# pymoc/pymoc

Measured on AMD Instinct MI355X. Metric: column-timesteps/sec (ensemble) at nz=100, higher is better.
Workload: dtype f64; 1 GPU; BASELINE configs[1]: 1024 independent Columns x nz=100 fp64 per GPU, static wA, do_conv on odd members, dt=30 d (pymoc_amd.configs.config2); columns_per_gpu=1024, nz=100, kernel=k_column_steps<64,2,6,true,true>, parallelism=ensemble sharded over 1 GPU(s), RCCL gather (root) of the final state

## Files before the change

### pymoc_amd/csrc/column.hip.h

```cpp
#pragma once
#include <type_traits>
#include "common.hip.h"

namespace pm {

template <int P>
struct ColGrid {
  double z[P];
  double dz[P];
  double dzc[P];
  double rdz[P], rdzc[P];
  double rdz_l[P], rdzc_l[P];
};
template <int P>
struct ColRegs {
  double b[P];
  double kap[P];
  double area[P];
  double dAk[P];
  double rarea[P];
  double rarea_l[P];
  double area_u, rarea_u, rarea_lu;
};

template <int P>
__device__ __forceinline__ void load_levels(double (&out)[P], const double *__restrict__ row,
                                            int lg, int nz, int lvl0 = 0) {
  if constexpr (P == 2) {
    if (lvl0 == 0 && (nz & 1) == 0 && (((unsigned long long)row) & 15ull) == 0ull) {
      const int i0 = lg * 2 < nz - 2 ? lg * 2 : nz - 2;
      const double2 v = *reinterpret_cast<const double2 *>(row + i0);
      out[0] = v.x;
      out[1] = v.y;
      return;
    }
  }
#pragma unroll
  for (int p = 0; p < P; ++p) {
    const int i = lvl0 + lg * P + p;
    out[p] = row[i < nz ? i : nz - 1];
  }
}

template <int P>
__device__ __forceinline__ double level_value(const double (&x)[P], int j) {
  const int jl = __builtin_amdgcn_readfirstlane(j / P);
  const int jp = __builtin_amdgcn_readfirstlane(j % P);
  double out = 0.;
#pragma unroll
  for (int p = 0; p < P; ++p) {
    const int lo = __builtin_amdgcn_readlane(__double2loint(x[p]), jl);
    const int hi = __builtin_amdgcn_readlane(__double2hiint(x[p]), jl);
    const double v = __hiloint2double(hi, lo);
    out = (p == 0 || jp == p) ? v : out;
  }
  return out;
}

__device__ __forceinline__ double lane_value(double x, int lane) {
  const int lo = __builtin_amdgcn_readlane(__double2loint(x), lane);
  const int hi = __builtin_amdgcn_readlane(__double2hiint(x), lane);
  return __hiloint2double(hi, lo);
}

template <int P>
struct ConvCache {
  unsigned long long mask[P];
  double zconv;
  bool valid = false;
};

template <int G, int P>
__device__ __forceinline__ bool col_convect(double (&b)[P], const double (&z)[P],
                                            double bs, double N2min, int lg, int lane,
                                            int nz, const double *__restrict__ zg,
                                            ConvCache<P> *cache = nullptr) {
  const unsigned long long gm = group_mask<G>(lane);
  bool ind[P];
  unsigned long long im[P];
  unsigned long long anym = 0ull;
#pragma unroll
  for (int p = 0; p < P; ++p) {
    const int i = lg * P + p;
    ind[p] = (i < nz) && (b[p] > bs);
    im[p] = __builtin_amdgcn_ballot_w64(ind[p]);
    anym |= im[p] & gm;
  }
  if (__builtin_expect(anym != 0ull, 0)) {
    double zconv;
    bool hit = false;
    if constexpr (G == 64) {
      if (cache != nullptr && cache->valid) {
        hit = true;
#pragma unroll
        for (int p = 0; p < P; ++p) hit = hit && (cache->mask[p] == im[p]);
      }
    }
    if (hit) {
      zconv = cache->zconv;
    } else {
      int jmax = 0;
#pragma unroll
      for (int p = 0; p < P; ++p) {
        const int i = lg * P + p;
        const unsigned long long m = __builtin_amdgcn_ballot_w64((i < nz) && !ind[p]) & gm;
        if (m != 0ull) {
          const int hl = 63 - __clzll((long long)m);
          const int j = (hl % G) * P + p;
          jmax = j > jmax ? j : jmax;
        }
      }
      if constexpr (G == 64) {
        zconv = level_value<P>(z, jmax);
        if (cache != nullptr) {
#pragma unroll
          for (int p = 0; p < P; ++p) cache->mask[p] = im[p];
          cache->zconv = zconv;
          cache->valid = true;
        }
      } else {
        zconv = zg[jmax];
      }
    }
#pragma unroll
    for (int p = 0; p < P; ++p) {
      const double adj = bs + N2min * (z[p] - zconv);
      b[p] = ind[p] ? adj : b[p];
    }
    return true;
  }
#pragma unroll
  for (int p = 0; p < P; ++p)
    if (lg * P + p == nz - 1) b[p] = bs;
  return false;
}

template <int P>
__device__ __forceinline__ void col_convect_cached(double (&b)[P], const double (&z)[P],
                                                   double bs, double N2min, int lane, int nz,
                                                   ConvCache<P> &cc) {
  bool ind[P];
  unsigned long long im[P], anym = 0ull;
  bool same = cc.valid;
#pragma unroll
  for (int p = 0; p < P; ++p) {
    ind[p] = (lane * P + p < nz) && (b[p] > bs);
    im[p] = __builtin_amdgcn_ballot_w64(ind[p]);
    anym |= im[p];
    same = same && (im[p] == cc.mask[p]);
  }
  if (__builtin_expect(!same, 0)) {
    int jmax = 0;
#pragma unroll
    for (int p = 0; p < P; ++p) {
      const unsigned long long m = __builtin_amdgcn_ballot_w64((lane * P + p < nz) && !ind[p]);
      if (m != 0ull) {
        const int j = (63 - __clzll((long long)m)) * P + p;
        jmax = j > jmax ? j : jmax;
      }
    }
    cc.zconv = level_value<P>(z, jmax);
#pragma unroll
    for (int p = 0; p < P; ++p) cc.mask[p] = im[p];
    cc.valid = true;
  }
  const bool none = anym == 0ull;
#pragma unroll
  for (int p = 0; p < P; ++p) {
    const double adj = bs + N2min * (z[p] - cc.zconv);
    b[p] = ind[p] ? adj : b[p];
    if (lane * P + p == nz - 1) b[p] = none ? bs : b[p];
  }
}

template <int G, int P, int DIV, bool BC = true, bool WEFF = false, bool UA = false,
          bool FLUXFMA = (DIV == 2 || DIV >= 6)>
__device__ __forceinline__ void col_vertadvdiff(const ColGrid<P> &g, ColRegs<P> &r,
                                                const double (&wA)[P],
                                                double dt, bool do_conv, double bs,
                                                double bbot, bool use_bzbot,
                                                double bzbot, int lg, int nz,
                                                int lvl0 = 0) {
  if (BC && !do_conv) {
#pragma unroll
    for (int p = 0; p < P; ++p)
      if (lvl0 + lg * P + p == nz - 1) r.b[p] = bs;
  }
  const double nb0 = from_next_lane_z(r.b[0]);
  double bup[P];
#pragma unroll
  for (int p = 0; p < P; ++p) bup[p] = (p < P - 1) ? r.b[p + 1 < P ? p + 1 : p] : nb0;
  if (BC && lvl0 + lg * P == 0) r.b[0] = use_bzbot ? (bup[0] - bzbot * g.dz[0]) : bbot;

  if constexpr (DIV == 4) {
    double d_up[P];
#pragma unroll
    for (int p = 0; p < P; ++p) d_up[p] = bup[p] - r.b[p];
    const double pd = from_prev_lane_z(d_up[P - 1]);
#pragma unroll
    for (int p = 0; p < P; ++p) {
      const double d_dn = (p > 0) ? d_up[p > 0 ? p - 1 : 0] : pd;
      r.b[p] = __builtin_fma(r.kap[p], d_up[p], __builtin_fma(r.dAk[p], d_dn, r.b[p]));
    }
    return;
  }
  double bz[P];
  {
    double num[P], q[P], rr[P];
#pragma unroll
    for (int p = 0; p < P; ++p) num[p] = bup[p] - r.b[p];
    if constexpr (DIV == 2) {
#pragma unroll
      for (int p = 0; p < P; ++p) rr[p] = num[p] * g.rdz_l[p];
#pragma unroll
      for (int p = 0; p < P; ++p) q[p] = __builtin_fma(num[p], g.rdz[p], rr[p]);
#pragma unroll
      for (int p = 0; p < P; ++p) rr[p] = __builtin_fma(-g.dz[p], q[p], num[p]);
#pragma unroll
      for (int p = 0; p < P; ++p) q[p] = __builtin_fma(rr[p], g.rdz[p], q[p]);
    } else if constexpr (DIV == 7 || DIV == 8) {
#pragma unroll
      for (int p = 0; p < P; ++p) rr[p] = num[p] * g.rdz_l[p];
#pragma unroll
      for (int p = 0; p < P; ++p) q[p] = __builtin_fma(num[p], g.rdz[p], rr[p]);
    } else if constexpr (DIV == 6) {
#pragma unroll
      for (int p = 0; p < P; ++p) q[p] = num[p] * g.rdz[p];
#pragma unroll
      for (int p = 0; p < P; ++p) rr[p] = __builtin_fma(-g.dz[p], q[p], num[p]);
#pragma unroll
      for (int p = 0; p < P; ++p) q[p] = __builtin_fma(rr[p], g.rdz[p], q[p]);
    } else if constexpr (DIV == 1 || DIV == 3 || DIV == 5) {
#pragma unroll
      for (int p = 0; p < P; ++p) q[p] = num[p] * g.rdz[p];
#pragma unroll
      for (int p = 0; p < P; ++p) rr[p] = __builtin_fma(-g.dz[p], q[p], num[p]);
#pragma unroll
      for (int p = 0; p < P; ++p) q[p] = __builtin_fma(rr[p], g.rdz[p], q[p]);
#pragma unroll
      for (int p = 0; p < P; ++p) rr[p] = __builtin_fma(-g.dz[p], q[p], num[p]);
#pragma unroll
      for (int p = 0; p < P; ++p) q[p] = __builtin_fma(rr[p], g.rdz[p], q[p]);
    } else {
#pragma unroll
      for (int p = 0; p < P; ++p) q[p] = num[p] / g.dz[p];
    }
    if constexpr (DIV != 0) {
#pragma unroll
      for (int p = 0; p < P; ++p) bz[p] = q[p];
    } else {
#pragma unroll
      for (int p = 0; p < P; ++p) bz[p] = (lvl0 + lg * P + p < nz - 1) ? q[p] : 0.0;
    }
  }
  const double pbz = from_prev_lane_z(bz[P - 1]);
  double bz_dn[P], dbz[P], flx[P], bzz[P], adv[P];
#pragma unroll
  for (int p = 0; p < P; ++p) {
    bz_dn[p] = (p > 0) ? bz[p > 0 ? p - 1 : 0] : pbz;
    dbz[p] = bz[p] - bz_dn[p];
    const double weff = WEFF ? wA[p] : wA[p] - r.dAk[p];
    if constexpr (FLUXFMA) {
      const double wn = (weff < 0.0) ? -weff : 0.0, wp = (weff < 0.0) ? 0.0 : -weff;
      flx[p] = __builtin_fma(wn, bz[p], wp * bz_dn[p]);
    } else {
      const double bzu = (weff < 0.0) ? bz[p] : bz_dn[p];
      flx[p] = (-weff) * bzu;
    }
  }
  if constexpr (DIV == 2) {
    double r1[P], r2[P];
#pragma unroll
    for (int p = 0; p < P; ++p) {
      r1[p] = dbz[p] * g.rdzc_l[p];
      r2[p] = flx[p] * (UA ? r.rarea_lu : r.rarea_l[p]);
    }
#pragma unroll
    for (int p = 0; p < P; ++p) {
      bzz[p] = __builtin_fma(dbz[p], g.rdzc[p], r1[p]);
      adv[p] = __builtin_fma(flx[p], (UA ? r.rarea_u : r.rarea[p]), r2[p]);
    }
#pragma unroll
    for (int p = 0; p < P; ++p) {
      r1[p] = __builtin_fma(-g.dzc[p], bzz[p], dbz[p]);
      r2[p] = __builtin_fma(-(UA ? r.area_u : r.area[p]), adv[p], flx[p]);
    }
#pragma unroll
    for (int p = 0; p < P; ++p) {
      bzz[p] = __builtin_fma(r1[p], g.rdzc[p], bzz[p]);
      adv[p] = __builtin_fma(r2[p], (UA ? r.rarea_u : r.rarea[p]), adv[p]);
    }
  } else if constexpr (DIV == 6) {
    double r1[P], r2[P];
#pragma unroll
    for (int p = 0; p < P; ++p) {
      bzz[p] = dbz[p] * g.rdzc[p];
      adv[p] = flx[p] * (UA ? r.rarea_u : r.rarea[p]);
    }
#pragma unroll
    for (int p = 0; p < P; ++p) {
      r1[p] = __builtin_fma(-g.dzc[p], bzz[p], dbz[p]);
      r2[p] = __builtin_fma(-(UA ? r.area_u : r.area[p]), adv[p], flx[p]);
    }
#pragma unroll
    for (int p = 0; p < P; ++p) {
      bzz[p] = __builtin_fma(r1[p], g.rdzc[p], bzz[p]);
      adv[p] = __builtin_fma(r2[p], (UA ? r.rarea_u : r.rarea[p]), adv[p]);
    }
  } else if constexpr (DIV == 8) {
    double r1[P], r2[P];
#pragma unroll
    for (int p = 0; p < P; ++p) {
      r1[p] = dbz[p] * g.rdzc_l[p];
      r2[p] = flx[p] * (UA ? r.rarea_lu : r.rarea_l[p]);
    }
#pragma unroll
    for (int p = 0; p < P; ++p) {
      bzz[p] = __builtin_fma(dbz[p], g.rdzc[p], r1[p]);
      adv[p] = __builtin_fma(flx[p], (UA ? r.rarea_u : r.rarea[p]), r2[p]);
    }
  } else if constexpr (DIV == 7) {
    double r1[P], r2[P];
#pragma unroll
    for (int p = 0; p < P; ++p) {
      r1[p] = dbz[p] * g.rdzc_l[p];
      adv[p] = flx[p] * (UA ? r.rarea_u : r.rarea[p]);
    }
#pragma unroll
    for (int p = 0; p < P; ++p) {
      bzz[p] = __builtin_fma(dbz[p], g.rdzc[p], r1[p]);
      r2[p] = __builtin_fma(-(UA ? r.area_u : r.area[p]), adv[p], flx[p]);
    }
#pragma unroll
    for (int p = 0; p < P; ++p) adv[p] = __builtin_fma(r2[p], (UA ? r.rarea_u : r.rarea[p]), adv[p]);
  } else if constexpr (DIV == 5) {
    double r1[P];
#pragma unroll
    for (int p = 0; p < P; ++p) {
      bzz[p] = dbz[p] * g.rdzc[p];
      adv[p] = div_by_recip2(flx[p], r.area_u, r.rarea_u, r.rarea_lu);
    }
#pragma unroll
    for (int k = 0; k < 2; ++k) {
#pragma unroll
      for (int p = 0; p < P; ++p) r1[p] = __builtin_fma(-g.dzc[p], bzz[p], dbz[p]);
#pragma unroll
      for (int p = 0; p < P; ++p) bzz[p] = __builtin_fma(r1[p], g.rdzc[p], bzz[p]);
    }
  } else if constexpr (DIV == 3) {
    double r1[P];
#pragma unroll
    for (int p = 0; p < P; ++p) {
      bzz[p] = dbz[p] * g.rdzc[p];
      adv[p] = flx[p] / (UA ? r.area_u : r.area[p]);
    }
#pragma unroll
    for (int k = 0; k < 2; ++k) {
#pragma unroll
      for (int p = 0; p < P; ++p) r1[p] = __builtin_fma(-g.dzc[p], bzz[p], dbz[p]);
#pragma unroll
      for (int p = 0; p < P; ++p) bzz[p] = __builtin_fma(r1[p], g.rdzc[p], bzz[p]);
    }
  } else if constexpr (DIV == 1) {
    double r1[P], r2[P];
#pragma unroll
    for (int p = 0; p < P; ++p) {
      bzz[p] = dbz[p] * g.rdzc[p];
      adv[p] = flx[p] * (UA ? r.rarea_u : r.rarea[p]);
    }
#pragma unroll
    for (int k = 0; k < 2; ++k) {
#pragma unroll
      for (int p = 0; p < P; ++p) {
        r1[p] = __builtin_fma(-g.dzc[p], bzz[p], dbz[p]);
        r2[p] = __builtin_fma(-(UA ? r.area_u : r.area[p]), adv[p], flx[p]);
      }
#pragma unroll
      for (int p = 0; p < P; ++p) {
        bzz[p] = __builtin_fma(r1[p], g.rdzc[p], bzz[p]);
        adv[p] = __builtin_fma(r2[p], (UA ? r.rarea_u : r.rarea[p]), adv[p]);
      }
    }
  } else {
#pragma unroll
    for (int p = 0; p < P; ++p) {
      bzz[p] = dbz[p] / g.dzc[p];
      adv[p] = flx[p] / (UA ? r.area_u : r.area[p]);
    }
  }
#pragma unroll
  for (int p = 0; p < P; ++p) {
    const int i = lvl0 + lg * P + p;
    const bool interior = (i >= 1) && (i <= nz - 2);
    const double db_dt = adv[p] + r.kap[p] * bzz[p];
    if constexpr (DIV == 0) {
      const double nb = r.b[p] + dt * db_dt;
      r.b[p] = interior ? nb : r.b[p];
    } else {
      r.b[p] = r.b[p] + (interior ? dt : 0.0) * db_dt;
    }
  }
}

template <int P>
__device__ __forceinline__ void col_horadv(ColRegs<P> &r, const double (&vdx)[P],
                                           const double (&bin)[P], double dt, int lg,
                                           int nz) {
#pragma unroll
  for (int p = 0; p < P; ++p) {
    const int i = lg * P + p;
    if (i < nz && vdx[p] > 0.0) {
      const double db = bin[p] - r.b[p];
      r.b[p] = r.b[p] + dt * vdx[p] * db / r.area[p];
    }
  }
}

template <int P>
__device__ __forceinline__ bool col_inputs_in_fast_range(const ColGrid<P> &g, const ColRegs<P> &r,
                                                         const double (&wA)[P], double dt,
                                                         double bs, double bbot, double bzbot,
                                                         double N2min, int lg, int nz) {
  bool ok = in_fast_div_range(dt) && in_fast_div_range(bs) && in_fast_div_range(bbot) &&
            in_fast_div_range(bzbot) && in_fast_div_range(N2min);
#pragma unroll
  for (int p = 0; p < P; ++p) {
    const bool top = lg * P + p >= nz - 1;
    ok = ok && in_fast_div_range(r.b[p]) && in_fast_div_range(wA[p]) &&
         in_fast_div_range(r.dAk[p]) && in_fast_div_range(wA[p] - r.dAk[p]) &&
         in_fast_div_range(r.kap[p]) && in_fast_div_range(r.area[p]) && r.area[p] != 0.0 &&
         in_fast_div_range(g.z[p]) && (top || (in_fast_div_range(g.dz[p]) && g.dz[p] != 0.0)) &&
         in_fast_div_range(g.dzc[p]) && g.dzc[p] != 0.0;
  }
  return ok;
}

template <int P>
__device__ __forceinline__ bool col_state_in_fast_range(const ColRegs<P> &r, const double (&wA)[P]) {
  int ok = 1;
#pragma unroll
  for (int p = 0; p < P; ++p)
    ok &= (int)in_fast_div_range(r.b[p]) & (int)in_fast_div_range(wA[p] - r.dAk[p]);
  return ok != 0;
}

template <int P, int DIV = 1>
__device__ __forceinline__ void col_load_grid(ColGrid<P> &g, const pm_columns &c, int lg,
                                              int lvl0 = 0) {
  const int nz = c.nz;
#pragma unroll
  for (int p = 0; p < P; ++p) {
    const int i = lvl0 + lg * P + p;
    const int ic = i < nz ? i : nz - 1;
    const int iu = ic + 1 < nz ? ic + 1 : nz - 1;
    const int id = ic > 0 ? ic - 1 : 0;
    const double zc = c.z[ic];
    g.z[p] = zc;
    g.dz[p] = c.z[iu] - zc;
    g.dzc[p] = 0.5 * (g.dz[p] + (zc - c.z[id]));
    if constexpr (DIV != 0 && DIV != 4) {
      g.rdz[p] = (i < nz - 1) ? 1.0 / g.dz[p] : 0.0;
      g.rdzc[p] = 1.0 / g.dzc[p];
    } else {
      g.rdz[p] = g.rdzc[p] = 0.0;
    }
    if constexpr (DIV == 2) {
      g.rdz_l[p] = (i < nz - 1) ? recip_lo(g.dz[p], g.rdz[p]) : 0.0;
      g.rdzc_l[p] = recip_lo(g.dzc[p], g.rdzc[p]);
    } else {
      g.rdz_l[p] = g.rdzc_l[p] = 0.0;
    }
  }
}

template <int P, int DIV = 1>
__device__ __forceinline__ void col_load_static(ColRegs<P> &r, const pm_columns &c,
                                                int col, int sel, int lg, int lvl0 = 0,
                                                bool uniform_area = false, bool weff_in = false) {
  const int nz = c.nz;
  const size_t base = (size_t)col * nz;
  const size_t sbase = ((size_t)sel * c.ncols + col) * nz;
  load_levels<P>(r.kap, c.kappa + sbase, lg, nz, lvl0);
  if (!weff_in) {
    load_levels<P>(r.dAk, c.dAkappa + sbase, lg, nz, lvl0);
  } else {
#pragma unroll
    for (int p = 0; p < P; ++p) r.dAk[p] = 0.0;
  }
  if (uniform_area) {
    const double a0 = c.area[base];
    const double ra = (DIV != 0 && DIV != 4) ? 1.0 / a0 : 0.0;
    const double ral = DIV == 2 ? recip_lo(a0, ra) : 0.0;
#pragma unroll
    for (int p = 0; p < P; ++p) {
      r.area[p] = a0;
      r.rarea[p] = ra;
      r.rarea_l[p] = ral;
    }
    return;
  }
  load_levels<P>(r.area, c.area + base, lg, nz, lvl0);
#pragma unroll
  for (int p = 0; p < P; ++p) {
    r.rarea[p] = (DIV != 0 && DIV != 4) ? 1.0 / r.area[p] : 0.0;
    r.rarea_l[p] = DIV == 2 ? recip_lo(r.area[p], r.rarea[p]) : 0.0;
  }
}

template <int P>
__device__ __forceinline__ void col_make_contracted(const ColGrid<P> &g, ColRegs<P> &r,
                                                    const double (&wA)[P], double dt, int lane,
                                                    int nz) {
  const double dz_prev_lane = from_prev_lane_z(g.dz[P - 1]);
#pragma unroll
  for (int p = 0; p < P; ++p) {
    const int i = lane * P + p;
    const bool interior = i >= 1 && i <= nz - 2;
    const double weff = wA[p] - r.dAk[p];
    const double dz_up = interior ? g.dz[p] : 1.0;
    const double dz_dn = interior ? ((p > 0) ? g.dz[p > 0 ? p - 1 : 0] : dz_prev_lane) : 1.0;
    const double dzc = interior ? g.dzc[p] : 1.0, area = interior ? r.area[p] : 1.0;
    const double wn = (weff < 0.0) ? -weff : 0.0, wp = (weff < 0.0) ? 0.0 : -weff;
    const double cu = dt * (r.kap[p] / (dzc * dz_up) + wn / (area * dz_up));
    const double cl = dt * (-r.kap[p] / (dzc * dz_dn) + wp / (area * dz_dn));
    r.kap[p] = interior ? cu : 0.0;
    r.dAk[p] = interior ? cl : 0.0;
  }
}

template <int P>
__device__ __forceinline__ unsigned conv_variant(const ConvCache<P> &cc) {
  unsigned need = 0u;
#pragma unroll
  for (int p = 0; p < P; ++p) need |= (cc.mask[p] != 0ull) ? (1u << p) : 0u;
  if constexpr (P <= 2) {
    return need;
  } else {
    return need ? (1u << P) - 1u : 0u;
  }
}

template <int P, int DIV, unsigned SEL, bool UA = false>
__device__ __forceinline__ int conv_spec_run(const ColGrid<P> &g, ColRegs<P> &r,
                                             const double (&wA)[P], double dt, double bs,
                                             double bbot, double N2min, int lane, int nz,
                                             ConvCache<P> &cc, int s, int nsteps) {
  constexpr int UNR = P <= 2 ? 16 : (P <= 4 ? 2 : 1);
  double adjv[P];
  double bs_eff[P];
  auto set_adj = [&]() {
#pragma unroll
    for (int p = 0; p < P; ++p)
      adjv[p] = (lane * P + p == 0) ? bbot : bs + N2min * (g.z[p] - cc.zconv);
  };
  set_adj();
#pragma unroll
  for (int p = 0; p < P; ++p) bs_eff[p] = (lane * P + p < nz) ? bs : __builtin_inf();
  double b_blk[P];
  unsigned long long acc;
  double bmax[P];
  auto spec = [&]() {
    unsigned long long im[P];
    bool ind[P];
#pragma unroll
    for (int p = 0; p < P; ++p) {
      if (((SEL >> p) & 1u) != 0u) {
        ind[p] = r.b[p] > bs_eff[p];
        im[p] = __builtin_amdgcn_ballot_w64(ind[p]);
      } else {
        bmax[p] = __builtin_fmax(bmax[p], r.b[p]);
      }
    }
#pragma unroll
    for (int p = 0; p < P; ++p) {
      if (((SEL >> p) & 1u) != 0u) r.b[p] = ind[p] ? adjv[p] : r.b[p];
    }
    col_vertadvdiff<64, P, DIV, false, false, UA>(g, r, wA, dt, true, bs, bbot, false, 0., lane, nz);
#pragma unroll
    for (int p = 0; p < P; ++p) {
      if (((SEL >> p) & 1u) != 0u) {
        unsigned long long x;
        asm("s_xor_b64 %0, %1, %2" : "=s"(x) : "s"(im[p]), "s"(cc.mask[p]) : "scc");
        acc |= x;
      }
    }
  };
  auto block_begin = [&]() {
    acc = 0ull;
#pragma unroll
    for (int p = 0; p < P; ++p) {
      b_blk[p] = r.b[p];
      bmax[p] = -__builtin_inf();
    }
  };
  auto block_bad = [&]() -> bool {
    bool conv = false;
#pragma unroll
    for (int p = 0; p < P; ++p)
      if (((SEL >> p) & 1u) == 0u) conv = conv || (bmax[p] > bs_eff[p]);
    if constexpr (SEL != (1u << P) - 1u) {
      unsigned long long any = __builtin_amdgcn_ballot_w64(conv);
      asm("" : "+s"(any));
      acc |= any;
    }
    return acc != 0ull;
  };
  auto redo = [&](int nb) {
#pragma unroll
    for (int p = 0; p < P; ++p) r.b[p] = b_blk[p];
    for (int k = 0; k < nb; ++k) {
      col_convect_cached<P>(r.b, g.z, bs, N2min, lane, nz, cc);
      if (lane == 0) r.b[0] = bbot;
      col_vertadvdiff<64, P, DIV, false, false, UA>(g, r, wA, dt, true, bs, bbot, false, 0., lane, nz);
    }
  };
  int pos = s, ret = -1;
  auto tier = [&](auto U) {
    constexpr int N = decltype(U)::value;
    int left = (nsteps - pos) / N;
    const int s_end = pos + left * N;
    for (; left > 0; --left) {
      block_begin();
#pragma unroll
      for (int k = 0; k < N; ++k) spec();
      if (__builtin_expect(block_bad(), 0)) {
        redo(N);
        if (conv_variant<P>(cc) != SEL) {
          ret = s_end - (left - 1) * N;
          left = 1;
        } else {
          set_adj();
        }
      }
    }
    pos = s_end;
  };
  if (UNR <= 4 || nsteps - pos >= 4 * UNR) tier(std::integral_constant<int, UNR>{});
  if (ret >= 0) return ret;
  if constexpr (UNR > 4) {
    tier(std::integral_constant<int, 4>{});
    if (ret >= 0) return ret;
  }
  if constexpr (UNR > 1) tier(std::integral_constant<int, 1>{});
  return ret >= 0 ? ret : nsteps;
}

template <int G, int P>
__device__ __forceinline__ void col_store_result(const pm_columns &c, const ColRegs<P> &r,
                                                 size_t base, int col, bool col_ok, int lg,
                                                 int lane, int nz) {
  bool bad = false;
  bool stored = false;
  if constexpr (P == 2) {
    if ((nz & 1) == 0 && (((unsigned long long)(c.b + base)) & 15ull) == 0ull) {
      if (lg * 2 < nz) {
        if (col_ok) *reinterpret_cast<double2 *>(c.b + base + lg * 2) = make_double2(r.b[0], r.b[1]);
        bad = !isfinite(r.b[0]) || !isfinite(r.b[1]);
      }
      stored = true;
    }
  }
  if (!stored) {
#pragma unroll
    for (int p = 0; p < P; ++p) {
      const int i = lg * P + p;
      if (i < nz) {
        if (col_ok) c.b[base + i] = r.b[p];
        bad |= !isfinite(r.b[p]);
      }
    }
  }
  if (c.nonfinite) {
    const unsigned long long m = __ballot(bad) & group_mask<G>(lane);
    if (lg == 0 && col_ok) c.nonfinite[col] = (m != 0ull) ? 1 : 0;
  }
}

template <int P>
__device__ __forceinline__ void col_pin(double (&b)[P]) {
#pragma unroll
  for (int p = 0; p < P; ++p) asm volatile("" : "+v"(b[p]));
}

template <int G, int P, int FAST, bool PLAIN, bool UA = false>
__global__ __launch_bounds__(256) void k_column_steps(
    pm_columns c, const double *__restrict__ wA_g, const double *__restrict__ vdx_g,
    const double *__restrict__ bin_g, double dt, int nsteps, int ops) {
  const int lane = threadIdx.x & (WAVE - 1);
  const int lg = threadIdx.x % G;
  int col_raw = (int)((blockIdx.x * (unsigned)blockDim.x + threadIdx.x) / G);
  constexpr bool FORMS = FAST == 6 && G == 64 && P <= 2 && PLAIN;
  if constexpr (FORMS) col_raw = __builtin_amdgcn_readfirstlane(col_raw);
  const bool col_ok = col_raw < c.ncols;
  const int col = col_ok ? col_raw : c.ncols - 1;
  const int nz = c.nz;
  const size_t base = (size_t)col * nz;

  ColGrid<P> g;
  ColRegs<P> r;
  const int sel = c.ksel ? c.ksel[col] : 0;
  const int flags = c.flags ? c.flags[col] : 0;
  col_load_grid<P, FAST>(g, c, lg);
  const bool ua = G == 64 && __builtin_amdgcn_readfirstlane(flags & PM_COL_UNIFORM_AREA) != 0;
  col_load_static<P, FAST>(r, c, col, sel, lg, 0, ua, (ops & PM_OP_WEFF) != 0);
  if constexpr (UA) {
    r.area_u = lane_value(r.area[0], 0);
    r.rarea_u = lane_value(r.rarea[0], 0);
    r.rarea_lu = lane_value(r.rarea_l[0], 0);
  }

  double wA[P], vdx[P], bin[P];
  load_levels<P>(r.b, c.b + base, lg, nz);
#pragma unroll
  for (int p = 0; p < P; ++p) wA[p] = vdx[p] = bin[p] = 0.0;
  const bool wA_row = !(PLAIN && (ops & PM_OP_WA_TWOBASIN) != 0 && col >= 2 * (c.ncols / 3));
  if (wA_g && wA_row) load_levels<P>(wA, wA_g + base, lg, nz);
  if constexpr (PLAIN) {
    if (ops & PM_OP_WA_PSI) {
      const int half = c.ncols >> 1;
      if (col < half) {
        if (bin_g) {
          double pso[P];
          load_levels<P>(pso, bin_g + base, lg, nz);
#pragma unroll
          for (int p = 0; p < P; ++p) wA[p] = (wA[p] - pso[p]) * 1e6;
        } else {
#pragma unroll
          for (int p = 0; p < P; ++p) wA[p] = wA[p] * 1e6;
        }
      } else {
#pragma unroll
        for (int p = 0; p < P; ++p) wA[p] = (-wA[p]) * 1e6;
      }
    }
  }
  if constexpr (PLAIN) {
    if (ops & PM_OP_WA_TWOBASIN) {
      const int third = c.ncols / 3;
      if (col < third) {
        double zon[P], pso[P];
        load_levels<P>(zon, vdx_g + base, lg, nz);
        load_levels<P>(pso, bin_g + base, lg, nz);
#pragma unroll
        for (int p = 0; p < P; ++p) wA[p] = (wA[p] + zon[p] - pso[p]) * 1e6;
      } else if (col < 2 * third) {
#pragma unroll
        for (int p = 0; p < P; ++p) wA[p] = (-wA[p]) * 1e6;
      } else {
        const size_t bp = (size_t)(col - third) * nz;
        double zon[P], pso[P];
        load_levels<P>(zon, vdx_g + bp, lg, nz);
        load_levels<P>(pso, bin_g + bp, lg, nz);
#pragma unroll
        for (int p = 0; p < P; ++p) wA[p] = (-zon[p] - pso[p]) * 1e6;
      }
    }
  }
  const bool wa_formed = (ops & (PM_OP_WA_PSI | PM_OP_WA_TWOBASIN)) != 0;
  if (vdx_g && !wa_formed) load_levels<P>(vdx, vdx_g + base, lg, nz);
  if (bin_g && !wa_formed) load_levels<P>(bin, bin_g + base, lg, nz);
  const bool do_conv = (flags & PM_COL_DO_CONV) != 0;
  const bool use_bzbot = (flags & PM_COL_BZBOT) != 0 && c.bzbot != nullptr;
  const double bs = c.bs[col];
  const double bbot = c.bbot[col];
  const double bzbot = use_bzbot ? c.bzbot[col] : 0.0;
  const double N2min = c.N2min[col];

  if constexpr (FAST != 0) {
    const bool vouched = G == 64 &&
                         __builtin_amdgcn_readfirstlane(flags & PM_COL_STATIC_IN_RANGE) != 0 &&
                         in_fast_div_range(dt);
    bool fast_ok;
    if (vouched)
      fast_ok = col_state_in_fast_range<P>(r, wA);
    else
      fast_ok = col_inputs_in_fast_range<P>(g, r, wA, dt, bs, bbot, bzbot, N2min, lg, nz);
    if (__builtin_expect(__ballot(!fast_ok) != 0ull, 0)) {
      for (int s = 0; s < nsteps; ++s) {
        if ((ops & PM_OP_CONVECT) && do_conv)
          col_convect<G, P>(r.b, g.z, bs, N2min, lg, lane, nz, c.z);
        col_pin<P>(r.b);
        if (ops & PM_OP_VERTADVDIFF)
          col_vertadvdiff<G, P, 0>(g, r, wA, dt, do_conv, bs, bbot, use_bzbot, bzbot, lg, nz);
        if ((ops & PM_OP_HORADV) && vdx_g) col_horadv<P>(r, vdx, bin, dt, lg, nz);
      }
      col_store_result<G, P>(c, r, base, col, col_ok, lg, lane, nz);
      return;
    }
  }

  if constexpr (FAST == 4) col_make_contracted<P>(g, r, wA, dt, lane, nz);

  auto plain_run = [&](auto DIVC) {
    constexpr int DIV = decltype(DIVC)::value;
    if (do_conv && use_bzbot) {
      for (int s = 0; s < nsteps; ++s) {
        col_convect<G, P>(r.b, g.z, bs, N2min, lg, lane, nz, c.z);
        col_vertadvdiff<G, P, DIV, true, false, UA>(g, r, wA, dt, true, bs, bbot, true, bzbot, lg, nz);
      }
    } else if (do_conv) {
      ConvCache<P> cc;
#pragma unroll
      for (int p = 0; p < P; ++p) cc.mask[p] = 0ull;
      cc.zconv = 0.;
      if constexpr (G == 64) {
        col_convect_cached<P>(r.b, g.z, bs, N2min, lane, nz, cc);
        if (lg == 0) r.b[0] = bbot;
        col_vertadvdiff<G, P, DIV, false, false, UA>(g, r, wA, dt, true, bs, bbot, false, 0., lg, nz);
        int s = 1;
        while (s < nsteps) {
          const unsigned v = conv_variant<P>(cc);
          if constexpr (P <= 2) {
            switch (v) {
              case 0: s = conv_spec_run<P, DIV, 0u, UA>(g, r, wA, dt, bs, bbot, N2min, lane, nz, cc, s, nsteps); break;
              case 1: s = conv_spec_run<P, DIV, 1u, UA>(g, r, wA, dt, bs, bbot, N2min, lane, nz, cc, s, nsteps); break;
              case 2: s = conv_spec_run<P, DIV, 2u, UA>(g, r, wA, dt, bs, bbot, N2min, lane, nz, cc, s, nsteps); break;
              default: s = conv_spec_run<P, DIV, 3u, UA>(g, r, wA, dt, bs, bbot, N2min, lane, nz, cc, s, nsteps); break;
            }
          } else {
            if (v == 0u)
              s = conv_spec_run<P, DIV, 0u, UA>(g, r, wA, dt, bs, bbot, N2min, lane, nz, cc, s, nsteps);
            else
              s = conv_spec_run<P, DIV, (1u << P) - 1u, UA>(g, r, wA, dt, bs, bbot, N2min, lane, nz, cc, s, nsteps);
          }
        }
      } else {
        for (int s = 0; s < nsteps; ++s) {
          col_convect<G, P>(r.b, g.z, bs, N2min, lg, lane, nz, c.z);
          if (lg == 0) r.b[0] = bbot;
          col_vertadvdiff<G, P, DIV, false, false, UA>(g, r, wA, dt, true, bs, bbot, false, 0., lg, nz);
        }
      }
    } else if (use_bzbot) {
      for (int s = 0; s < nsteps; ++s)
        col_vertadvdiff<G, P, DIV, true, false, UA>(g, r, wA, dt, false, bs, bbot, true, bzbot, lg, nz);
    } else {
#pragma unroll
      for (int p = 0; p < P; ++p) {
        if (lg * P + p == nz - 1) r.b[p] = bs;
        if (lg * P + p == 0) r.b[p] = bbot;
      }
      int s = 0;
      if constexpr (P <= 2) {
        for (; s + 4 <= nsteps; s += 4) {
          col_vertadvdiff<G, P, DIV, false, false, UA>(g, r, wA, dt, false, bs, bbot, false, 0., lg, nz);
          col_vertadvdiff<G, P, DIV, false, false, UA>(g, r, wA, dt, false, bs, bbot, false, 0., lg, nz);
          col_vertadvdiff<G, P, DIV, false, false, UA>(g, r, wA, dt, false, bs, bbot, false, 0., lg, nz);
          col_vertadvdiff<G, P, DIV, false, false, UA>(g, r, wA, dt, false, bs, bbot, false, 0., lg, nz);
        }
      }
      for (; s < nsteps; ++s)
        col_vertadvdiff<G, P, DIV, false, false, UA>(g, r, wA, dt, false, bs, bbot, false, 0., lg, nz);
    }
  };
  if constexpr (PLAIN) {
    if constexpr (FORMS) {
      const bool d2g = (c.reserved & PM_COLS_DIV3_PROVEN) != 0 && (c.reserved & PM_COLS_DIV2_GRID) != 0;
      if (d2g) {
#pragma unroll
        for (int p = 0; p < P; ++p) {
          const bool below_top = lg * P + p < nz - 1;
          g.rdz_l[p] = below_top ? recip_lo_div(g.dz[p], g.rdz[p]) : 0.0;
          g.rdzc_l[p] = below_top ? recip_lo_div(g.dzc[p], g.rdzc[p]) : 0.0;
        }
        if (__builtin_amdgcn_readfirstlane(flags & PM_COL_DIV2_AREA) != 0) {
          if constexpr (UA) {
            r.rarea_lu = lane_value(recip_lo_div(r.area_u, r.rarea_u), 0);
          } else {
#pragma unroll
            for (int p = 0; p < P; ++p) r.rarea_l[p] = recip_lo_div(r.area[p], r.rarea[p]);
          }
          plain_run(std::integral_constant<int, 8>{});
        } else {
          plain_run(std::integral_constant<int, 7>{});
        }
      } else {
        plain_run(std::integral_constant<int, 6>{});
      }
    } else {
      plain_run(std::integral_constant<int, FAST>{});
    }
  } else {
    for (int s = 0; s < nsteps; ++s) {
      if ((ops & PM_OP_CONVECT) && do_conv)
        col_convect<G, P>(r.b, g.z, bs, N2min, lg, lane, nz, c.z);
      col_pin<P>(r.b);
      if (ops & PM_OP_VERTADVDIFF)
        col_vertadvdiff<G, P, FAST, true, false, UA>(g, r, wA, dt, do_conv, bs, bbot, use_bzbot, bzbot, lg, nz);
      if ((ops & PM_OP_HORADV) && vdx_g) col_horadv<P>(r, vdx, bin, dt, lg, nz);
    }
  }

  col_store_result<G, P>(c, r, base, col, col_ok, lg, lane, nz);
}

template <int P>
struct ColStage {
  double b[P], wA[P], kap[P], area[P], dAk[P];
};
template <int P>
struct ColStageLean {
  double b[P], wA[P];
};

struct StreamScalars {
  int flags, sel;
  double bs, bbot, bzbot, N2min, area0, kbase;
  double ra, ral;
  __device__ __forceinline__ void load(const pm_columns &c, int col0, int cend, int lane) {
    const int col = col0 + lane < cend ? col0 + lane : cend - 1;
    flags = c.flags ? c.flags[col] : 0;
    sel = c.ksel ? c.ksel[col] : 0;
    bs = c.bs[col];
    bbot = c.bbot[col];
    N2min = c.N2min[col];
    bzbot = ((flags & PM_COL_BZBOT) != 0 && c.bzbot != nullptr) ? c.bzbot[col] : 0.0;
    area0 = (flags & PM_COL_UNIFORM_AREA) ? c.area[(size_t)col * c.nz] : 0.0;
    kbase = c.kappa_base ? c.kappa_base[col] : 0.0;
    ra = 1.0 / area0;
    ral = recip_lo(area0, ra);
  }
};

template <int P, bool AFF = false>
__device__ __forceinline__ void col_stage_load(ColStage<P> &s, const pm_columns &c,
                                               const double *__restrict__ wA_g, int col,
                                               int lane, bool weff_in, int flags, int sel,
                                               double area0) {
  const int nz = c.nz;
  const size_t base = (size_t)col * nz;
  const size_t sbase = ((size_t)sel * c.ncols + col) * nz;
  load_levels<P>(s.b, c.b + base, lane, nz);
  load_levels<P>(s.wA, wA_g + base, lane, nz);
  if constexpr (!AFF) load_levels<P>(s.kap, c.kappa + sbase, lane, nz);
  if ((flags & PM_COL_UNIFORM_AREA) == 0) {
    load_levels<P>(s.area, c.area + base, lane, nz);
  } else {
#pragma unroll
    for (int p = 0; p < P; ++p) s.area[p] = area0;
  }
  if (!weff_in) {
    load_levels<P>(s.dAk, c.dAkappa + sbase, lane, nz);
  } else {
#pragma unroll
    for (int p = 0; p < P; ++p) s.dAk[p] = 0.0;
  }
}

template <int P, int D, bool AFF = false, bool LEAN = false, bool VEC = false, bool D3 = false,
          int CPWU = 0, int WEFFT = -1, int UABT = -1>
__global__ __launch_bounds__(256) __attribute__((amdgpu_waves_per_eu((LEAN && P <= 2 && D <= 5) ? 4 : 1)))
void k_column_stream(pm_columns c,
                                                       const double *__restrict__ wA_g,
                                                       double dt, int nsteps, int cpw, bool dt_ok,
                                                       bool weff_in) {
  const int lane = threadIdx.x & (WAVE - 1);
  const int wave = (int)((blockIdx.x * (unsigned)blockDim.x + threadIdx.x) >> 6);
  const int col0 = __builtin_amdgcn_readfirstlane(wave * cpw);
  const int nz = c.nz;
  if (col0 >= c.ncols) return;
  const int cend = col0 + cpw < c.ncols ? col0 + cpw : c.ncols;

  StreamScalars sc;
  sc.load(c, col0, cend, lane);
  static_assert(!LEAN || AFF, "the lean ring needs the affine kappa");
  static_assert(!VEC || (LEAN && P == 2), "16-byte accesses: the lean form with two levels per lane");
  const int off2 = lane * 2 < nz - 2 ? lane * 2 : nz - 2;
  using Stage = typename std::conditional<LEAN, ColStageLean<P>, ColStage<P>>::type;
  auto flags_of = [&](int k) { return __builtin_amdgcn_readlane(sc.flags, k); };
  auto issue = [&](Stage &st, int col) {
    const int k = col - col0;
    if constexpr (VEC) {
      const size_t base = (size_t)col * nz;
      const double2 vb = *reinterpret_cast<const double2 *>(c.b + base + off2);
      const double2 vw = *reinterpret_cast<const double2 *>(wA_g + base + off2);
      st.b[0] = vb.x;
      st.b[P - 1] = vb.y;
      st.wA[0] = vw.x;
      st.wA[P - 1] = vw.y;
    } else if constexpr (LEAN) {
      const size_t base = (size_t)col * nz;
      load_levels<P>(st.b, c.b + base, lane, nz);
      load_levels<P>(st.wA, wA_g + base, lane, nz);
    } else if constexpr (CPWU > 0 && WEFFT >= 0 && UABT >= 0) {
      const int sel = __builtin_amdgcn_readlane(sc.sel, k);
      const size_t base = (size_t)col * nz, sbase = ((size_t)sel * c.ncols + col) * nz;
      load_levels<P>(st.b, c.b + base, lane, nz);
      load_levels<P>(st.wA, wA_g + base, lane, nz);
      if constexpr (!AFF) load_levels<P>(st.kap, c.kappa + sbase, lane, nz);
      if constexpr (UABT == 0) load_levels<P>(st.area, c.area + base, lane, nz);
      if constexpr (WEFFT == 0) load_levels<P>(st.dAk, c.dAkappa + sbase, lane, nz);
    } else {
      col_stage_load<P, AFF>(st, c, wA_g, col, lane, weff_in, flags_of(k),
                             __builtin_amdgcn_readlane(sc.sel, k), lane_value(sc.area0, k));
    }
  };
  ColGrid<P> g;
  col_load_grid<P, 1>(g, c, lane);
  double kprof[P];
#pragma unroll
  for (int p = 0; p < P; ++p) kprof[p] = 0.0;
  if constexpr (AFF) load_levels<P>(kprof, c.kappa_profile, lane, nz);
  Stage ring[D];
#pragma unroll
  for (int d = 0; d < D; ++d)
    if (col0 + d < cend) issue(ring[d], col0 + d);
  unsigned nf_bits = 0u;
  auto one_column = [&](int col, int d, bool prefetch, int kk) {
      ColRegs<P> r;
      double wA[P];
#pragma unroll
      for (int p = 0; p < P; ++p) {
        r.b[p] = ring[d].b[p];
        wA[p] = ring[d].wA[p];
        if constexpr (AFF)
          r.kap[p] = lane_value(sc.kbase, col - col0) + kprof[p];
        else
          r.kap[p] = ring[d].kap[p];
        if constexpr (LEAN) {
          r.area[p] = lane_value(sc.area0, col - col0);
          r.area_u = r.area[p];
          r.rarea_u = lane_value(sc.ra, col - col0);
          r.rarea_lu = lane_value(sc.ral, col - col0);
          r.dAk[p] = 0.0;
        } else if constexpr (CPWU > 0 && WEFFT >= 0 && UABT >= 0) {
          if constexpr (UABT == 1)
            r.area[p] = lane_value(sc.area0, col - col0);
          else
            r.area[p] = ring[d].area[p];
          if constexpr (WEFFT == 1)
            r.dAk[p] = 0.0;
          else
            r.dAk[p] = ring[d].dAk[p];
        } else {
          r.area[p] = ring[d].area[p];
          r.dAk[p] = ring[d].dAk[p];
        }
        r.rarea[p] = r.rarea_l[p] = 0.;
      }
      if (CPWU > 0) {
        if (prefetch) issue(ring[d], col + D);
      } else {
        issue(ring[d], col + D < cend ? col + D : cend - 1);
      }
      const int k = col - col0;
      const int flags = flags_of(k);
      const bool do_conv = (flags & PM_COL_DO_CONV) != 0;
      const bool use_bzbot = (flags & PM_COL_BZBOT) != 0 && c.bzbot != nullptr;
      const double bs = lane_value(sc.bs, k), bbot = lane_value(sc.bbot, k),
                   N2min = lane_value(sc.N2min, k), bzbot = lane_value(sc.bzbot, k);
      const bool fast_ok = ((flags & PM_COL_STATIC_IN_RANGE) != 0 && dt_ok)
                               ? col_state_in_fast_range<P>(r, wA)
                               : col_inputs_in_fast_range<P>(g, r, wA, dt, bs, bbot, bzbot, N2min,
                                                             lane, nz);
      const bool slow = __ballot(!fast_ok) != 0ull;
      for (int s = 0; s < nsteps; ++s) {
        if (do_conv) col_convect<64, P>(r.b, g.z, bs, N2min, lane, lane, nz, c.z);
        col_pin<P>(r.b);
        if (__builtin_expect(slow, 0))
          col_vertadvdiff<64, P, 0>(g, r, wA, dt, do_conv, bs, bbot, use_bzbot, bzbot, lane, nz);
        else if constexpr (LEAN && D3)
          col_vertadvdiff<64, P, 6, true, false, true, false>(g, r, wA, dt, do_conv, bs, bbot, use_bzbot,
                                                              bzbot, lane, nz);
        else if constexpr (LEAN)
          col_vertadvdiff<64, P, 5, true, false, true>(g, r, wA, dt, do_conv, bs, bbot, use_bzbot,
                                                       bzbot, lane, nz);
        else
          col_vertadvdiff<64, P, 3>(g, r, wA, dt, do_conv, bs, bbot, use_bzbot, bzbot, lane, nz);
      }
      const size_t base = (size_t)col * nz;
      bool bad = false;
      bool stored = false;
      if constexpr (VEC) {
        if (lane * 2 < nz) {
          *reinterpret_cast<double2 *>(c.b + base + lane * 2) = make_double2(r.b[0], r.b[P - 1]);
          bad = !isfinite(r.b[0]) || !isfinite(r.b[P - 1]);
        }
        stored = true;
      } else if constexpr (P == 2) {
        if ((nz & 1) == 0 && (((unsigned long long)(c.b + base)) & 15ull) == 0ull) {
          if (lane * 2 < nz) {
            *reinterpret_cast<double2 *>(c.b + base + lane * 2) = make_double2(r.b[0], r.b[1]);
            bad = !isfinite(r.b[0]) || !isfinite(r.b[1]);
          }
          stored = true;
        }
      }
      if (!stored) {
#pragma unroll
        for (int p = 0; p < P; ++p) {
          const int i = lane * P + p;
          if (i < nz) {
            c.b[base + i] = r.b[p];
            bad |= !isfinite(r.b[p]);
          }
        }
      }
      if (CPWU > 0) {
        nf_bits |= (__ballot(bad) != 0ull ? 1u : 0u) << kk;
      } else if (c.nonfinite) {
        const unsigned long long m = __ballot(bad);
        if (lane == 0) c.nonfinite[col] = (m != 0ull) ? 1 : 0;
      }
  };
  if constexpr (CPWU > 0) {
#pragma unroll
    for (int k = 0; k < CPWU; ++k) one_column(col0 + k, k % D, k + D < CPWU, k);
    if (c.nonfinite && lane < CPWU) c.nonfinite[col0 + lane] = (int)((nf_bits >> lane) & 1u);
  } else {
    for (int colb = col0; colb < cend; colb += D) {
#pragma unroll
      for (int d = 0; d < D; ++d) {
        const int col = colb + d;
        if (col >= cend) break;
        one_column(col, d, true, 0);
      }
    }
  }
}

inline int stream_cols_per_wave(int ncols) {
  const int waves_wanted = 1024 * 8;
  int cpw = ncols / waves_wanted;
  return cpw < 1 ? 1 : (cpw > 32 ? 32 : cpw);
}

inline int pick_levels_per_lane(int G, int need) {
  static const int sup64[] = {1, 2, 3, 4, 5, 6, 7, 8, 10, 13, 16};
  static const int sup[] = {1, 2, 3, 4, 5, 6, 7, 8};
  if (G == 64) {
    for (int v : sup64)
      if (v >= need) return v;
  } else {
    for (int v : sup)
      if (v >= need) return v;
  }
  return -1;
}

struct ColKernel {
  bool stream, plain, ua, aff, lean, vec, d3;
  int fast, d, cpwu, wefft, uabt;
  constexpr bool compiled(int G, int P) const {
    if (!stream && !ua && fast <= 2) return true;
    return G == 64 && P <= 4 && (P == 2 || (!vec && cpwu == 0));
  }
};
constexpr ColKernel col_steps(int fast, bool plain, bool ua = false) {
  return {false, plain, ua, false, false, false, false, fast, 0, 0, -1, -1};
}
constexpr ColKernel col_stream(int d, bool aff = false, bool lean = false, bool vec = false,
                               bool d3 = false, int cpwu = 0, int wefft = -1, int uabt = -1) {
  return {true, false, false, aff, lean, vec, d3, 0, d, cpwu, wefft, uabt};
}

#define PM_COLUMN_KERNELS(X)                                                                   \
  X(CK_STEPS_IEEE, col_steps(0, false))                                         \
  X(CK_STEPS_RECIP, col_steps(1, false))              \
  X(CK_STEPS_PLAIN, col_steps(2, true))                              \
  X(CK_STEPS_PLAIN_UA, col_steps(2, true, true))                \
  X(CK_STEPS_DIV3_UA, col_steps(6, true, true))           \
  X(CK_STEPS_CONTRACTED, col_steps(4, true))                         \
  X(CK_STREAM, col_stream(2))                                \
  X(CK_STREAM_WEFF, col_stream(3))                                    \
  X(CK_STREAM_AFF, col_stream(3, true))                 \
  X(CK_STREAM_WEFF_AFF, col_stream(4, true))                                                   \
  X(CK_STREAM_LEAN, col_stream(5, true, true))            \
  X(CK_STREAM_LEAN_VEC, col_stream(5, true, true, true))             \
  X(CK_STREAM_LEAN_VEC_D3, col_stream(5, true, true, true, true))                              \
  X(CK_STREAM_LEAN_VEC_U8, col_stream(5, true, true, true, false, 8))       \
  X(CK_STREAM_LEAN_VEC_D3_U8, col_stream(5, true, true, true, true, 8))                        \
  X(CK_STREAM_U8, col_stream(2, false, false, false, false, 8, 0, 0))                          \
  X(CK_STREAM_WEFF_UA_U8, col_stream(3, false, false, false, false, 8, 1, 1))

#define PM_CK_ID(id, args) id,
enum ColKernelId { CK_NONE, PM_COLUMN_KERNELS(PM_CK_ID) };
#undef PM_CK_ID
constexpr ColKernel col_kernel(ColKernelId k) {
#define PM_CK_ARGS(id, args) \
  case id: return args;
  switch (k) {
    PM_COLUMN_KERNELS(PM_CK_ARGS)
    default: return {};
  }
#undef PM_CK_ARGS
}

struct ColumnPlan {
  ColKernelId kernel;
  int G, P;
  int cpw;
  unsigned grid;
};

inline ColumnPlan column_plan(const pm_columns &c, const double *wA, const double *vdx, int nsteps,
                              int ops, int G, int P) {
  const bool weff = (ops & PM_OP_WEFF) != 0;
  const bool plain =
      (ops & ~(PM_OP_WEFF | PM_OP_CONTRACTED | PM_OP_WA_PSI | PM_OP_WA_TWOBASIN)) == PM_OP_TIMESTEP &&
      (!vdx || (ops & PM_OP_WA_TWOBASIN));
  const bool ua = (c.reserved & PM_COLS_ALL_UNIFORM_AREA) != 0;
  const bool d3 = (c.reserved & PM_COLS_DIV3_PROVEN) != 0;
  const bool aff = c.kappa_base && c.kappa_profile && c.nsel == 1;
  const bool wave_per_col = G == 64 && P <= 4;
  const int cpw = stream_cols_per_wave(c.ncols);
  ColumnPlan pl{CK_STEPS_IEEE, G, P, 0, (unsigned)((c.ncols + 256 / G - 1) / (256 / G))};
  if (wave_per_col && nsteps < 3 && plain && cpw >= 2) {
    pl.cpw = cpw;
    if (weff && aff && ua) {
      pl.cpw = c.ncols / 16384 < 2 ? 2 : (c.ncols / 16384 > 16 ? 16 : c.ncols / 16384);
      const bool vec = P == 2 && (c.nz & 1) == 0 &&
                       ((((unsigned long long)c.b) | ((unsigned long long)wA)) & 15ull) == 0ull;
      const bool u8 = vec && c.ncols % 8 == 0 && c.ncols >= 8 * 4096;
      if (u8) pl.cpw = 8;
      pl.kernel = !vec ? CK_STREAM_LEAN
                  : u8 ? (d3 ? CK_STREAM_LEAN_VEC_D3_U8 : CK_STREAM_LEAN_VEC_U8)
                       : (d3 ? CK_STREAM_LEAN_VEC_D3 : CK_STREAM_LEAN_VEC);
    } else if (P == 2 && !aff && c.ncols % 8 == 0 && c.ncols >= 8 * 4096 && weff == ua) {
      pl.cpw = 8;
      pl.kernel = weff ? CK_STREAM_WEFF_UA_U8 : CK_STREAM_U8;
    } else {
      pl.kernel = weff ? (aff ? CK_STREAM_WEFF_AFF : CK_STREAM_WEFF) : (aff ? CK_STREAM_AFF : CK_STREAM);
    }
    const unsigned waves = (unsigned)((c.ncols + pl.cpw - 1) / pl.cpw);
    pl.grid = (waves + 3) / 4;
  } else if (nsteps >= 3 && plain) {
    if (wave_per_col && (ops & PM_OP_CONTRACTED))
      pl.kernel = CK_STEPS_CONTRACTED;
    else if (wave_per_col && ua)
      pl.kernel = d3 ? CK_STEPS_DIV3_UA : CK_STEPS_PLAIN_UA;
    else
      pl.kernel = CK_STEPS_PLAIN;
  } else if (nsteps >= 3) {
    pl.kernel = CK_STEPS_RECIP;
  }
  return pl;
}

inline int column_kernel_name(const ColumnPlan &pl, char *name, size_t len) {
  const ColKernel k = col_kernel(pl.kernel);
  auto tf = [](bool v) { return v ? "true" : "false"; };
  int n = 0;
  if (pl.kernel == CK_NONE)
    n = snprintf(name, len, "%s", "");
  else if (k.stream)
    n = snprintf(name, len, "k_column_stream<%d,%d,%s,%s,%s,%s,%d,%d,%d>", pl.P, k.d, tf(k.aff),
                 tf(k.lean), tf(k.vec), tf(k.d3), k.cpwu, k.wefft, k.uabt);
  else
    n = snprintf(name, len, "k_column_steps<%d,%d,%d,%s,%s>", pl.G, pl.P, k.fast, tf(k.plain),
                 tf(k.ua));
  PM_REQUIRE(n >= 0 && (size_t)n < len, "name buffer of %zu bytes too small", len);
  return PM_OK;
}

template <int G, int P, ColKernelId K>
int launch_column_kernel(const ColumnPlan &pl, const pm_columns &c, const double *wA,
                         const double *vdx, const double *bin, double dt, int nsteps, int ops,
                         hipStream_t st) {
  constexpr ColKernel k = col_kernel(K);
  if constexpr (!k.compiled(G, P)) {
    return fail(PM_EINVAL, "column kernel %d is not compiled for G=%d P=%d", (int)K, G, P);
  } else if constexpr (k.stream) {
    const double adt = dt < 0 ? -dt : dt;
    const bool dt_ok = dt == 0.0 || (adt >= 0x1p-200 && adt <= 0x1p200);
    hipLaunchKernelGGL((k_column_stream<P, k.d, k.aff, k.lean, k.vec, k.d3, k.cpwu, k.wefft, k.uabt>),
                       dim3(pl.grid), dim3(256), 0, st, c, wA, dt, nsteps, pl.cpw, dt_ok,
                       (ops & PM_OP_WEFF) != 0);
  } else {
    hipLaunchKernelGGL((k_column_steps<G, P, k.fast, k.plain, k.ua>), dim3(pl.grid), dim3(256), 0,
                       st, c, wA, vdx, bin, dt, nsteps, ops & ~PM_OP_CONTRACTED);
  }
  PM_HIP(hipGetLastError());
  return PM_OK;
}

template <int G, int P>
int launch_column_steps(const ColumnPlan &pl, const pm_columns &c, const double *wA,
                        const double *vdx, const double *bin, double dt, int nsteps, int ops,
                        hipStream_t st) {
#define PM_CK_LAUNCH(id, args) \
  case id: return launch_column_kernel<G, P, id>(pl, c, wA, vdx, bin, dt, nsteps, ops, st);
  switch (pl.kernel) {
    PM_COLUMN_KERNELS(PM_CK_LAUNCH)
    default: return PM_OK;
  }
#undef PM_CK_LAUNCH
}

int column_steps_g16(const ColumnPlan &pl, const pm_columns &c, const double *wA,
                     const double *vdx, const double *bin, double dt, int nsteps, int ops,
                     hipStream_t st);
int column_steps_g32(const ColumnPlan &pl, const pm_columns &c, const double *wA,
                     const double *vdx, const double *bin, double dt, int nsteps, int ops,
                     hipStream_t st);
int column_steps_g64(const ColumnPlan &pl, const pm_columns &c, const double *wA,
                     const double *vdx, const double *bin, double dt, int nsteps, int ops,
                     hipStream_t st);
int column_steps_implicit(const pm_columns &c, const double *wA, const double *zon,
                          const double *so, double dt, int nsteps, int ops, hipStream_t st);

}
```

Measured before the change: 13.85 billion column-timesteps/s.

## Add classified convection kernel with surface-only class and integer high-word filter

Adds a twin kernel, k_column_steps_cls, which is launched for G=64, P<=2, plain, uniform-area configs when nsteps>=64. Its speculative convection loop classifies columns whose only convective level is the surface, so that stable held value is checked by bit equality instead of triggering redo. When no level convects, it swaps the per-step fmax tracking for a cheaper integer max over the high word of each double, using a DPP shift for the paired-slot layout. The goal is to cut per-step detection cost and avoid spurious rollbacks, at the cost of more template variants, code size and register pressure, plus subtle correctness conditions on sign and exponent ranges.

```diff
diff --git a/pymoc_amd/csrc/column.hip.h b/pymoc_amd/csrc/column.hip.h
--- a/pymoc_amd/csrc/column.hip.h
+++ b/pymoc_amd/csrc/column.hip.h
@@ -540,14 +540,56 @@
   }
 }
 
-template <int P, int DIV, unsigned SEL, bool UA = false>
+constexpr unsigned CONV_SURF = 4u;
+template <int P>
+__device__ __forceinline__ bool conv_surface_only(const ConvCache<P> &cc, int nz) {
+  if constexpr (P <= 2) {
+    bool only = nz >= 2;
+    const int ls = (nz - 1) / P, ps = (nz - 1) % P;
+#pragma unroll
+    for (int p = 0; p < P; ++p) only = only && (cc.mask[p] == ((p == ps) ? (1ull << ls) : 0ull));
+    return only;
+  } else {
+    return false;
+  }
+}
+template <int P>
+__device__ __forceinline__ unsigned conv_class(const ConvCache<P> &cc, const double (&b)[P],
+                                               const double (&z)[P], double bs, double N2min,
+                                               int nz, long long &surf_bits) {
+  const unsigned need = conv_variant<P>(cc);
+  surf_bits = 0;
+  if constexpr (P <= 2) {
+    if (conv_surface_only<P>(cc, nz)) {
+      const double zs = level_value<P>(z, nz - 1), held = level_value<P>(b, nz - 1);
+      const double adj = bs + N2min * (zs - cc.zconv);
+      const bool is = adj > bs && __double_as_longlong(held) == __double_as_longlong(adj);
+      if (__builtin_amdgcn_ballot_w64(is) != 0ull) {
+        surf_bits = __double_as_longlong(lane_value(adj, 0));
+        return CONV_SURF;
+      }
+    }
+  }
+  return need;
+}
+
+struct ConvCls {
+  int surf = 0;
+  long long surf_bits = 0;
+  bool filt = false;
+};
+template <int P, int DIV, unsigned SEL, int IF, bool UA = false, bool CLS = false>
 __device__ __forceinline__ int conv_spec_run(const ColGrid<P> &g, ColRegs<P> &r,
                                              const double (&wA)[P], double dt, double bs,
                                              double bbot, double N2min, int lane, int nz,
-                                             ConvCache<P> &cc, int s, int nsteps) {
+                                             ConvCache<P> &cc, ConvCls &cls, int s, int nsteps) {
+  static_assert(IF == 0 || (CLS && P <= 2 && SEL == 0u), "the integer filter serves slots outside SEL");
+  constexpr bool SURFCLS = CLS && SEL == 0u && P <= 2;
+  static_assert(IF != 2 || P == 2, "the shifted operands pair two slots");
   constexpr int UNR = P <= 2 ? 16 : (P <= 4 ? 2 : 1);
   double adjv[P];
   double bs_eff[P];
+  const unsigned long long surf_mask = (unsigned long long)(long long)cls.surf;
   auto set_adj = [&]() {
 #pragma unroll
     for (int p = 0; p < P; ++p)
@@ -555,19 +597,29 @@
   };
   set_adj();
 #pragma unroll
-  for (int p = 0; p < P; ++p) bs_eff[p] = (lane * P + p < nz) ? bs : __builtin_inf();
+  for (int p = 0; p < P; ++p)
+    bs_eff[p] = (lane * P + p < nz) ? bs : __builtin_inf();
   double b_blk[P];
   unsigned long long acc;
   double bmax[P];
+  int imax;
   auto spec = [&]() {
     unsigned long long im[P];
     bool ind[P];
+    if constexpr (IF == 1) {
+      imax = imax > __double2hiint(r.b[0]) ? imax : __double2hiint(r.b[0]);
+      if constexpr (P == 2) imax = imax > __double2hiint(r.b[1]) ? imax : __double2hiint(r.b[1]);
+    } else if constexpr (IF == 2) {
+      const int nh = __builtin_amdgcn_update_dpp(0, __double2hiint(r.b[0]), 0x130, 0xf, 0xf, true);
+      imax = imax > nh ? imax : nh;
+      imax = imax > __double2hiint(r.b[1]) ? imax : __double2hiint(r.b[1]);
+    }
 #pragma unroll
     for (int p = 0; p < P; ++p) {
       if (((SEL >> p) & 1u) != 0u) {
         ind[p] = r.b[p] > bs_eff[p];
         im[p] = __builtin_amdgcn_ballot_w64(ind[p]);
-      } else {
+      } else if constexpr (IF == 0) {
         bmax[p] = __builtin_fmax(bmax[p], r.b[p]);
       }
     }
@@ -587,6 +639,7 @@
   };
   auto block_begin = [&]() {
     acc = 0ull;
+    imax = -__INT_MAX__ - 1;
 #pragma unroll
     for (int p = 0; p < P; ++p) {
       b_blk[p] = r.b[p];
@@ -595,10 +648,28 @@
   };
   auto block_bad = [&]() -> bool {
     bool conv = false;
-#pragma unroll
-    for (int p = 0; p < P; ++p)
-      if (((SEL >> p) & 1u) == 0u) conv = conv || (bmax[p] > bs_eff[p]);
-    if constexpr (SEL != (1u << P) - 1u) {
+    if constexpr (IF != 0) {
+      const int hb = __builtin_amdgcn_readfirstlane(__double2hiint(bs));
+      unsigned long long alarm = __builtin_amdgcn_ballot_w64(imax >= hb);
+      asm("" : "+s"(alarm));
+      acc |= alarm & ((1ull << ((nz - 1) / P)) - 1ull);
+    } else if constexpr (SURFCLS) {
+      const unsigned long long surf_lane = (1ull << ((nz - 1) / P)) & surf_mask;
+#pragma unroll
+      for (int p = 0; p < P; ++p) {
+        unsigned long long any = __builtin_amdgcn_ballot_w64(bmax[p] > bs_eff[p]);
+        asm("" : "+s"(any));
+        acc |= any & ~((p == (nz - 1) % P) ? surf_lane : 0ull);
+      }
+    } else {
+#pragma unroll
+      for (int p = 0; p < P; ++p)
+        if (((SEL >> p) & 1u) == 0u) conv = conv || (bmax[p] > bs_eff[p]);
+    }
+    if constexpr (SURFCLS) {
+      acc |= (unsigned long long)(__double_as_longlong(level_value<P>(r.b, nz - 1)) ^ cls.surf_bits) & surf_mask;
+    }
+    if constexpr (SEL != (1u << P) - 1u && !SURFCLS) {
       unsigned long long any = __builtin_amdgcn_ballot_w64(conv);
       asm("" : "+s"(any));
       acc |= any;
@@ -625,7 +696,16 @@
       for (int k = 0; k < N; ++k) spec();
       if (__builtin_expect(block_bad(), 0)) {
         redo(N);
-        if (conv_variant<P>(cc) != SEL) {
+        bool leave;
+        if constexpr (IF != 0) {
+          cls.filt = false;
+          leave = true;
+        } else if constexpr (CLS) {
+          leave = cls.surf != 0 || conv_variant<P>(cc) != SEL || conv_surface_only<P>(cc, nz);
+        } else {
+          leave = conv_variant<P>(cc) != SEL;
+        }
+        if (leave) {
           ret = s_end - (left - 1) * N;
           left = 1;
         } else {
@@ -682,9 +762,9 @@
   for (int p = 0; p < P; ++p) asm volatile("" : "+v"(b[p]));
 }
 
-template <int G, int P, int FAST, bool PLAIN, bool UA = false>
-__global__ __launch_bounds__(256) void k_column_steps(
-    pm_columns c, const double *__restrict__ wA_g, const double *__restrict__ vdx_g,
+template <int G, int P, int FAST, bool PLAIN, bool UA, bool CLS>
+__device__ __forceinline__ void column_steps_body(
+    const pm_columns &c, const double *__restrict__ wA_g, const double *__restrict__ vdx_g,
     const double *__restrict__ bin_g, double dt, int nsteps, int ops) {
   const int lane = threadIdx.x & (WAVE - 1);
   const int lg = threadIdx.x % G;
@@ -808,20 +888,49 @@
         if (lg == 0) r.b[0] = bbot;
         col_vertadvdiff<G, P, DIV, false, false, UA>(g, r, wA, dt, true, bs, bbot, false, 0., lg, nz);
         int s = 1;
-        while (s < nsteps) {
-          const unsigned v = conv_variant<P>(cc);
-          if constexpr (P <= 2) {
+        if constexpr (!CLS) {
+          while (s < nsteps) {
+            const unsigned v = conv_variant<P>(cc);
+            ConvCls cls;
+#define PM_SPEC(SEL) \
+  s = conv_spec_run<P, DIV, SEL, 0, UA>(g, r, wA, dt, bs, bbot, N2min, lane, nz, cc, cls, s, nsteps)
+            if constexpr (P <= 2) {
+              switch (v) {
+                case 0: PM_SPEC(0u); break;
+                case 1: PM_SPEC(1u); break;
+                case 2: PM_SPEC(2u); break;
+                default: PM_SPEC(3u); break;
+              }
+            } else {
+              if (v == 0u)
+                PM_SPEC(0u);
+              else
+                PM_SPEC((1u << P) - 1u);
+            }
+#undef PM_SPEC
+          }
+        } else {
+          static_assert(!CLS || (G == 64 && P <= 2), "the class loops exist for P <= 2");
+          ConvCls cls;
+          const unsigned hb = (unsigned)__builtin_amdgcn_readfirstlane(__double2hiint(bs));
+          cls.filt = hb - 0x00100000u < 0x7fe00000u && __builtin_amdgcn_ballot_w64(bbot > bs) == 0ull;
+          const bool shifted = P == 2 && (nz & 1) == 0;
+          while (s < nsteps) {
+            const unsigned v = conv_class<P>(cc, r.b, g.z, bs, N2min, nz, cls.surf_bits);
+            cls.surf = __builtin_amdgcn_readfirstlane(v == CONV_SURF ? -1 : 0);
+#define PM_SPEC(SEL, IF) \
+  s = conv_spec_run<P, DIV, SEL, IF, UA, true>(g, r, wA, dt, bs, bbot, N2min, lane, nz, cc, cls, s, nsteps)
             switch (v) {
-              case 0: s = conv_spec_run<P, DIV, 0u, UA>(g, r, wA, dt, bs, bbot, N2min, lane, nz, cc, s, nsteps); break;
-              case 1: s = conv_spec_run<P, DIV, 1u, UA>(g, r, wA, dt, bs, bbot, N2min, lane, nz, cc, s, nsteps); break;
-              case 2: s = conv_spec_run<P, DIV, 2u, UA>(g, r, wA, dt, bs, bbot, N2min, lane, nz, cc, s, nsteps); break;
-              default: s = conv_spec_run<P, DIV, 3u, UA>(g, r, wA, dt, bs, bbot, N2min, lane, nz, cc, s, nsteps); break;
+              case 1: PM_SPEC(1u, 0); break;
+              case 2: PM_SPEC(P == 2 ? 2u : 1u, 0); break;
+              case 3: PM_SPEC(P == 2 ? 3u : 1u, 0); break;
+              default:
+                if (!cls.filt) PM_SPEC(0u, 0);
+                else if (shifted) PM_SPEC(0u, P == 2 ? 2 : 1);
+                else PM_SPEC(0u, 1);
+                break;
             }
-          } else {
-            if (v == 0u)
-              s = conv_spec_run<P, DIV, 0u, UA>(g, r, wA, dt, bs, bbot, N2min, lane, nz, cc, s, nsteps);
-            else
-              s = conv_spec_run<P, DIV, (1u << P) - 1u, UA>(g, r, wA, dt, bs, bbot, N2min, lane, nz, cc, s, nsteps);
+#undef PM_SPEC
           }
         }
       } else {
@@ -892,6 +1001,19 @@
   }
 
   col_store_result<G, P>(c, r, base, col, col_ok, lg, lane, nz);
+}
+
+template <int G, int P, int FAST, bool PLAIN, bool UA = false>
+__global__ __launch_bounds__(256) void k_column_steps(
+    pm_columns c, const double *__restrict__ wA_g, const double *__restrict__ vdx_g,
+    const double *__restrict__ bin_g, double dt, int nsteps, int ops) {
+  column_steps_body<G, P, FAST, PLAIN, UA, false>(c, wA_g, vdx_g, bin_g, dt, nsteps, ops);
+}
+template <int G, int P, int FAST, bool PLAIN, bool UA>
+__global__ __launch_bounds__(256) void k_column_steps_cls(
+    pm_columns c, const double *__restrict__ wA_g, const double *__restrict__ vdx_g,
+    const double *__restrict__ bin_g, double dt, int nsteps, int ops) {
+  column_steps_body<G, P, FAST, PLAIN, UA, true>(c, wA_g, vdx_g, bin_g, dt, nsteps, ops);
 }
 
 template <int P>
@@ -1267,6 +1389,15 @@
                        dim3(pl.grid), dim3(256), 0, st, c, wA, dt, nsteps, pl.cpw, dt_ok,
                        (ops & PM_OP_WEFF) != 0);
   } else {
+    constexpr bool twin = G == 64 && P <= 2 && k.plain && k.ua;
+    if constexpr (twin) {
+      if (nsteps >= 64) {
+        hipLaunchKernelGGL((k_column_steps_cls<G, P, k.fast, k.plain, k.ua>), dim3(pl.grid), dim3(256),
+                           0, st, c, wA, vdx, bin, dt, nsteps, ops & ~PM_OP_CONTRACTED);
+        PM_HIP(hipGetLastError());
+        return PM_OK;
+      }
+    }
     hipLaunchKernelGGL((k_column_steps<G, P, k.fast, k.plain, k.ua>), dim3(pl.grid), dim3(256), 0,
                        st, c, wA, vdx, bin, dt, nsteps, ops & ~PM_OP_CONTRACTED);
   }
```

After: 14.82 billion column-timesteps/s, median of 6. 7.0% higher.
